# FelipeMartins96/rsoccer-isaac-cleanrl

Measured on AMD Instinct MI355X. Metric: env-steps/s (num_envs×horizon) at 65 536 envs; PPO wall-clock to 1e8 steps, higher is better.
Workload: dtype f32; 1 GPU; vss_step FULL contract: 65536 fields/GPU, one launch per control step, random actions (BASELINE configs[1]/[2] shape); fields_per_gpu=65536, mode=full, agent_rows_per_field=1, launch=eager ctypes launches, parallelism=fields sharded over 1 GPU(s), no data-path collective

## Files before the change

### rsoccer-isaac-cleanrl_amd/csrc/vss_step.hip

```cpp
#include <hip/hip_runtime.h>
#include <type_traits>
#include <stdint.h>

#include "../../include/vss.h"

#pragma clang fp contract(off)

#if defined(__HIP_DEVICE_COMPILE__) && !defined(__gfx950__)
#error "vss_step.hip targets gfx950 (CDNA4) only: wait_loads() and v_permlane32_swap are gfx950 encodings"
#endif

namespace vss {

constexpr int kWave = 64;
constexpr int kFpw = 32;
constexpr int kRec = 59;

constexpr int NSUB = 2;
#define K_H 0.025f
#define K_HH 0.0125f
#define K_FIELD_HX 0.75f
#define K_FIELD_HY 0.65f
#define K_GOAL_HY 0.2f
#define K_GOAL_BACK_X 0.85f
// ... 210 lines not shown
    float dx = ax - K_FIELD_HX, dy = ay - K_GOAL_HY;
    float d2 = dx * dx + dy * dy;
    if (d2 < r * r) {
      float d = sqrtf(d2);
      float nx = -1.0f, ny = 0.0f;
      if (d > 1e-9f) { float inv = 1.0f / d; nx = dx * inv; ny = dy * inv; }
      float pen = r - d;
      ax = ax + nx * pen; ay = ay + ny * pen;
      float vn = avx * nx + avy * ny;
      if (vn < 0.0f) { avx = avx - nx * vn; avy = avy - ny * vn; }
    }
  } else {
    const float px = ax - K_FIELD_HX + r, py = ay - K_GOAL_HY + r;
    const float pen_end = ax + r - K_FIELD_HX, pen_side = ay + r - K_GOAL_HY;
    const bool use_x = in_x || (!in_y && px < py);
    const float pen = in_x ? pen_end : (in_y ? pen_side : (px < py ? px : py));
    push_face(ax, avx, use_x ? pen : -1.0f);
    push_face(ay, avy, use_x ? -1.0f : pen);
  }
  push_face(ay, avy, ay + r - K_FIELD_HY);
  push_face(ax, avx, ax + r - K_GOAL_BACK_X);
  x = ax * sx; y = ay * sy; vx = avx * sx; vy = avy * sy;
}

__device__ __forceinline__ void drive_robot(float c, float s, float& vx, float& vy, float& w, float tl, float tr) {
  float vf = c * vx + s * vy;
  float vl = c * vy - s * vx;
  float wl = vf - w * K_HALF_TRACK;
  float wr = vf + w * K_HALF_TRACK;
  wl = wl + clampf(tl - wl, -K_DV, K_DV);
  wr = wr + clampf(tr - wr, -K_DV, K_DV);
  vf = (wl + wr) * 0.5f;
  w = (wr - wl) * K_INV_TRACK;
  vl = vl - clampf(vl, -K_DL, K_DL);
  vx = c * vf - s * vl;
  vy = s * vf + c * vl;
}

__device__ __forceinline__ void integrate_robot(float& x, float& y, float vx, float vy, float w, float& qz, float& qw,
                                                float& c, float& s) {
  x = x + vx * K_H;
  y = y + vy * K_H;
  float sh, ch;
  sincos_small(w * K_HH, sh, ch);
  const float nqz = qz * ch + qw * sh;
  const float nqw = qw * ch - qz * sh;
  const float k = 1.5f - 0.5f * (nqz * nqz + nqw * nqw);
  qz = nqz * k;
  qw = nqw * k;
  c = qw * qw - qz * qz;
  s = 2.0f * qw * qz;
}

__device__ __forceinline__ void exch(float v, float& lo, float& hi) {
  const auto r = __builtin_amdgcn_permlane32_swap(__float_as_uint(v), __float_as_uint(v), false, false);
  lo = __uint_as_float(r[0]);
  hi = __uint_as_float(r[1]);
}

__device__ __forceinline__ void physics_split(Bodies& b, const float a[12]) {
  const bool up = threadIdx.x >= 32;
  float tl[3], tr[3], ox[3], oy[3], ovx[3], ovy[3], ow[3], oqz[3], oqw[3], oc[3], os[3];
#pragma unroll
  for (int k = 0; k < 3; ++k) {
    const float al = up ? a[2 * k + 6] : a[2 * k], ar = up ? a[2 * k + 7] : a[2 * k + 1];
    tl[k] = (al * K_WHEEL_RAD_S) * K_WHEEL_R;
    tr[k] = (ar * K_WHEEL_RAD_S) * K_WHEEL_R;
    ox[k] = up ? b.x[k + 3] : b.x[k];
    oy[k] = up ? b.y[k + 3] : b.y[k];
    ovx[k] = up ? b.vx[k + 3] : b.vx[k];
    ovy[k] = up ? b.vy[k + 3] : b.vy[k];
    ow[k] = up ? b.w[k + 3] : b.w[k];
    oqz[k] = up ? b.qz[k + 3] : b.qz[k];
    oqw[k] = up ? b.qw[k + 3] : b.qw[k];
    oc[k] = oqw[k] * oqw[k] - oqz[k] * oqz[k];
    os[k] = 2.0f * oqw[k] * oqz[k];
  }
#pragma unroll 1
  for (int sub = 0; sub < NSUB; ++sub) {
#pragma unroll
    for (int k = 0; k < 3; ++k) {
      drive_robot(oc[k], os[k], ovx[k], ovy[k], ow[k], tl[k], tr[k]);
      integrate_robot(ox[k], oy[k], ovx[k], ovy[k], ow[k], oqz[k], oqw[k], oc[k], os[k]);
      exch(ox[k], b.x[k], b.x[k + 3]);
      exch(oy[k], b.y[k], b.y[k + 3]);
      exch(ovx[k], b.vx[k], b.vx[k + 3]);
      exch(ovy[k], b.vy[k], b.vy[k + 3]);
      exch(oc[k], b.c[k], b.c[k + 3]);
      exch(os[k], b.s[k], b.s[k + 3]);
    }
    b.bvx = b.bvx * K_BALL_DAMP;
    b.bvy = b.bvy * K_BALL_DAMP;
    b.bx = b.bx + b.bvx * K_H;
    b.by = b.by + b.bvy * K_H;
#pragma unroll
    for (int i = 0; i < 6; ++i)
#pragma unroll
      for (int j = i + 1; j < 6; ++j) contact_robot_robot(b, i, j);
#pragma unroll
    for (int i = 0; i < 6; ++i) contact_ball_robot(b, i);
#pragma unroll
    for (int k = 0; k < 3; ++k) {
      ox[k] = up ? b.x[k + 3] : b.x[k];
      oy[k] = up ? b.y[k + 3] : b.y[k];
      ovx[k] = up ? b.vx[k + 3] : b.vx[k];
      ovy[k] = up ? b.vy[k + 3] : b.vy[k];
      contact_walls(ox[k], oy[k], ovx[k], ovy[k], K_ROBOT_R);
      exch(ox[k], b.x[k], b.x[k + 3]);
      exch(oy[k], b.y[k], b.y[k + 3]);
      exch(ovx[k], b.vx[k], b.vx[k + 3]);
      exch(ovy[k], b.vy[k], b.vy[k + 3]);
    }
    contact_walls(b.bx, b.by, b.bvx, b.bvy, K_BALL_R);
  }
// ... 61 lines not shown
    const float2* g2 = reinterpret_cast<const float2*>(g);
    for (int q = lane; q < total / 2; q += kWave) {
      float2 v = at(g2, 8u * (uint32_t)q);
      int e = q * 2, fl = e / W, k = e - fl * W;
      float* d = lds + fl * kRec + k;
      d[0] = v.x; d[1] = v.y;
    }
  }
}

template <int W>
__device__ __forceinline__ void coop_store(float* __restrict__ g, int nv, const float* lds, int lane) {
  const int total = nv * W;
  if constexpr (W % 4 == 0) {
    float4* g4 = reinterpret_cast<float4*>(g);
    for (int q = lane; q < total / 4; q += kWave) {
      int e = q * 4, fl = e / W, k = e - fl * W;
      const float* s = lds + fl * kRec + k;
      at(g4, 16u * (uint32_t)q) = make_float4(s[0], s[1], s[2], s[3]);
    }
  } else {
    float2* g2 = reinterpret_cast<float2*>(g);
    for (int q = lane; q < total / 2; q += kWave) {
      int e = q * 2, fl = e / W, k = e - fl * W;
      const float* s = lds + fl * kRec + k;
      at(g2, 8u * (uint32_t)q) = make_float2(s[0], s[1]);
    }
  }
}

template <int A>
__device__ __forceinline__ void write_obs_record(float* rec, const Bodies& b, const float dof[12]) {
  rec[0] = b.bx; rec[1] = b.by; rec[2] = b.bvx; rec[3] = b.bvy;
#pragma unroll
  for (int r = 0; r < 6; ++r) {
    float* o = rec + 4 + 9 * r;
    o[0] = b.x[r]; o[1] = b.y[r]; o[2] = b.vx[r]; o[3] = b.vy[r];
    o[4] = b.qw[r] * b.qw[r] - b.qz[r] * b.qz[r];
    o[5] = 2.0f * b.qw[r] * b.qz[r];
    o[6] = b.w[r]; o[7] = dof[2 * r]; o[8] = dof[2 * r + 1];
  }
  if constexpr (A == 6) {
    float* m = rec + kRec;
#pragma unroll
    for (int k = 0; k < 4; ++k) m[k] = __uint_as_float(__float_as_uint(rec[k]) ^ 0x80000000u);
#pragma unroll
    for (int r = 0; r < 6; ++r)
#pragma unroll
      for (int q = 0; q < 6; ++q)
        m[4 + 6 * r + q] = __uint_as_float(__float_as_uint(rec[4 + 9 * r + q]) ^ 0x80000000u);
  }
}

constexpr int kObsUnroll = 4;
template <int A, int A0 = 0, int REC = obs_rec<A>()>
__device__ __forceinline__ void coop_store_obs(float* __restrict__ out, int nv, const float* lds, const uint32_t* tab,
                                               int lane, bool nt = false) {
  static_assert(A0 + A <= 6 && (A0 == 0 || REC == kRecObs6), "yellow agents read the mirror slots");
  constexpr int Q = 13 * A;
  constexpr int QD = kWave / Q, QR = kWave % Q;
  constexpr uint32_t RB = 4u * REC;
  const int total = nv * Q;
  const uint32_t rb_last = (uint32_t)(nv - 1) * RB;
  int fl = lane / Q, j4 = lane - fl * Q;
  uint32_t rb = (uint32_t)fl * RB;
  const char* L = reinterpret_cast<const char*>(lds);
  float4* o4 = reinterpret_cast<float4*>(out);
  for (int q0 = lane; q0 < total; q0 += kObsUnroll * kWave) {
    float4 v[kObsUnroll];
#pragma unroll
    for (int u = 0; u < kObsUnroll; ++u) {
      const uint2 t = reinterpret_cast<const uint2*>(tab)[13 * A0 + j4];
      const uint32_t r = rb < rb_last ? rb : rb_last;
      v[u].x = *reinterpret_cast<const float*>(L + r + (t.x & 0xffffu));
      v[u].y = *reinterpret_cast<const float*>(L + r + (t.x >> 16));
      v[u].z = *reinterpret_cast<const float*>(L + r + (t.y & 0xffffu));
      v[u].w = *reinterpret_cast<const float*>(L + r + (t.y >> 16));
      j4 += QR;
      rb += QD * RB;
      if (j4 >= Q) { j4 -= Q; rb += RB; }
    }
#pragma unroll
    for (int u = 0; u < kObsUnroll; ++u)
      if (q0 + u * kWave < total) {
        if (nt) {
          typedef float f4v __attribute__((ext_vector_type(4)));
          __builtin_nontemporal_store(f4v{v[u].x, v[u].y, v[u].z, v[u].w},
                                      reinterpret_cast<f4v*>(&at(o4, 16u * (uint32_t)(q0 + u * kWave))));
        } else {
          at(o4, 16u * (uint32_t)(q0 + u * kWave)) = v[u];
        }
      }
  }
}

struct ResetDraws {
  uint32_t k0, k1, field, ctr, ext;
  const float* u;
  uint32_t rounds;
};

template <bool REPLAY>
__device__ __forceinline__ float uval(uint32_t w) { return REPLAY ? __uint_as_float(w) : u01(w); }

template <bool REPLAY>
__device__ __forceinline__ void pos_block(const ResetDraws& d, uint32_t round, uint32_t blk, uint32_t o[4]) {
  if constexpr (REPLAY) {
#pragma unroll
    for (uint32_t i = 0; i < 4; ++i) {
      const uint32_t j = 4u * blk + i;
      o[i] = j < 14u ? __float_as_uint(d.u[14u * round + j]) : 0x3f000000u;
    }
  } else {
    philox(d.k0, d.k1, d.field, d.ctr, ((kPurposePos | d.ext) << 24) | round, blk, o);
  }
}

template <bool REPLAY>
__device__ __forceinline__ void ang_block(const ResetDraws& d, uint32_t rounds_used, uint32_t blk, uint32_t o[4]) {
  if constexpr (REPLAY) {
#pragma unroll
    for (uint32_t i = 0; i < 4; ++i) o[i] = __float_as_uint(d.u[14u * rounds_used + 4u * blk + i]);
  } else {
    philox(d.k0, d.k1, d.field, d.ctr, ((kPurposeAng | d.ext) << 24), blk, o);
  }
}

template <bool REPLAY>
__device__ __forceinline__ void reset_field(Bodies& b, const ResetDraws& d) {
  const float scale_x = 1.5f - 0.14f, scale_y = 1.3f - 0.14f;
  float px[7], py[7];
  uint32_t round = 0;
  for (;; ++round) {
    uint32_t o[16];
#pragma unroll
    for (int blk = 0; blk < 4; ++blk) pos_block<REPLAY>(d, round, (uint32_t)blk, o + 4 * blk);
#pragma unroll
    for (int e = 0; e < 7; ++e) {
      px[e] = (uval<REPLAY>(o[2 * e]) - 0.5f) * scale_x;
      py[e] = (uval<REPLAY>(o[2 * e + 1]) - 0.5f) * scale_y;
    }
    bool close = false;
#pragma unroll
    for (int i = 0; i < 7; ++i)
#pragma unroll
      for (int j = i + 1; j < 7; ++j) {
        float dx = px[i] - px[j], dy = py[i] - py[j];
        close |= dx * dx + dy * dy < __uint_as_float(0x3ba0902du);
      }
    if (!close || round + 1 >= d.rounds) break;
  }
  b.bx = px[0]; b.by = py[0];
  uint32_t o[8];
  ang_block<REPLAY>(d, round + 1, 0u, o);
  ang_block<REPLAY>(d, round + 1, 1u, o + 4);
#pragma unroll
  for (int r = 0; r < 6; ++r) {
    b.x[r] = px[1 + r]; b.y[r] = py[1 + r];
    b.vx[r] = 0.0f; b.vy[r] = 0.0f; b.w[r] = 0.0f;
    float ang = K_TWO_PI * uval<REPLAY>(o[r]) + (-K_PI);
    float sh, ch;
    sincos_small(ang * 0.5f, sh, ch);
    float nrm = sqrtf(sh * sh + ch * ch);
    b.qz[r] = sh / nrm;
    b.qw[r] = ch / nrm;
  }
  b.bvx = uval<REPLAY>(o[6]) - 0.5f;
  b.bvy = uval<REPLAY>(o[7]) - 0.5f;
}

template <bool REPLAY>
__device__ __forceinline__ void reset_field_split(Bodies& b, const ResetDraws& d) {
  const float kMinDist2 = __uint_as_float(0x3ba0902du);
  const bool up = threadIdx.x >= 32;
  const uint32_t blk0 = up ? 2u : 0u;
  const float scale_x = 1.5f - 0.14f, scale_y = 1.3f - 0.14f;
  float px[8], py[8];
  uint32_t round = 0;
  for (;; ++round) {
    uint32_t o[8];
    pos_block<REPLAY>(d, round, blk0, o);
    pos_block<REPLAY>(d, round, blk0 + 1u, o + 4);
#pragma unroll
    for (int e = 0; e < 4; ++e) {
      exch((uval<REPLAY>(o[2 * e]) - 0.5f) * scale_x, px[e], px[4 + e]);
      exch((uval<REPLAY>(o[2 * e + 1]) - 0.5f) * scale_y, py[e], py[4 + e]);
    }
    bool close = false;
#pragma unroll
    for (int i = 0; i < 7; ++i)
#pragma unroll
      for (int j = i + 1; j < 7; ++j) {
        float dx = px[i] - px[j], dy = py[i] - py[j];
        close |= dx * dx + dy * dy < kMinDist2;
      }
    if (!close || round + 1 >= d.rounds) break;
  }
  b.bx = px[0]; b.by = py[0];
  uint32_t oa[4], ang_u[8];
  ang_block<REPLAY>(d, round + 1, up ? 1u : 0u, oa);
#pragma unroll
  for (int i = 0; i < 4; ++i) {
    float lo, hi;
    exch(__uint_as_float(oa[i]), lo, hi);
    ang_u[i] = __float_as_uint(lo);
    ang_u[4 + i] = __float_as_uint(hi);
  }
#pragma unroll
  for (int k = 0; k < 3; ++k) {
    float ang = K_TWO_PI * uval<REPLAY>(up ? ang_u[k + 3] : ang_u[k]) + (-K_PI);
    float sh, ch;
    sincos_small(ang * 0.5f, sh, ch);
    float nrm = sqrtf(sh * sh + ch * ch);
    exch(sh / nrm, b.qz[k], b.qz[k + 3]);
    exch(ch / nrm, b.qw[k], b.qw[k + 3]);
  }
#pragma unroll
  for (int r = 0; r < 6; ++r) {
    b.x[r] = px[1 + r]; b.y[r] = py[1 + r];
    b.vx[r] = 0.0f; b.vy[r] = 0.0f; b.w[r] = 0.0f;
  }
  b.bvx = uval<REPLAY>(ang_u[6]) - 0.5f;
  b.bvy = uval<REPLAY>(ang_u[7]) - 0.5f;
}

__device__ __forceinline__ int64_t rewards_and_done(const vss_params& p, const Bodies& b, float pbx, float pby,
                                                   const float prx[6], const float pry[6], const float a[12],
                                                   int64_t progress, float rew[24]) {
  const float bx = b.bx, by = b.by;
  const bool is_goal = (fabsf(bx) > K_FIELD_HX) && (fabsf(by) < K_GOAL_HY);
  const float g = is_goal ? (bx > 0.0f ? 1.0f : (bx < 0.0f ? -1.0f : 0.0f)) : 0.0f;
  float grad;
  {
    float lx = bx - (-K_FIELD_HX), ly = by - (-0.0f), rx = bx - K_FIELD_HX, ry = by - 0.0f;
    float pot = sqrtf(lx * lx + ly * ly) - sqrtf(rx * rx + ry * ry);
    float plx = pbx - (-K_FIELD_HX), ply = pby - (-0.0f), prx_ = pbx - K_FIELD_HX, pry_ = pby - 0.0f;
    float ppot = sqrtf(plx * plx + ply * ply) - sqrtf(prx_ * prx_ + pry_ * pry_);
    grad = pot - ppot;
  }
#pragma unroll
  for (int ag = 0; ag < 6; ++ag) {
    const bool blue = ag < 3;
    float r0 = 0.0f, r1 = 0.0f, r2 = 0.0f, r3 = 0.0f;
    if (p.w_goal > 0.0f) r0 = (blue ? g : (0.0f - g)) * p.w_goal;
    if (p.w_grad > 0.0f) r1 = (blue ? grad : -grad) * p.w_grad;
    if (p.w_move > 0.0f) {
      float dx0 = prx[ag] - pbx, dy0 = pry[ag] - pby;
      float dx1 = b.x[ag] - bx, dy1 = b.y[ag] - by;
      float pd = sqrtf(dx0 * dx0 + dy0 * dy0), d = sqrtf(dx1 * dx1 + dy1 * dy1);
      r2 = 0.0f + (pd - d) * p.w_move;
    }
    if (p.w_energy > 0.0f)
      r3 = 0.0f + (-((fabsf(a[2 * ag]) + fabsf(a[2 * ag + 1])) / 2.0f)) * p.w_energy;
    rew[4 * ag] = r0; rew[4 * ag + 1] = r1; rew[4 * ag + 2] = r2; rew[4 * ag + 3] = r3;
  }
  return (is_goal || progress >= (int64_t)p.max_episode_length) ? 1 : 0;
}

__device__ __forceinline__ void prefetch12(const float* __restrict__ g, int nv, int lane, float4 pre[3]) {
  const float4* g4 = reinterpret_cast<const float4*>(g);
#pragma unroll
  for (int j = 0; j < 3; ++j) {
    const int q = lane + j * kWave;
    if (q < nv * 3) pre[j] = at(g4, 16u * (uint32_t)q);
  }
}

__device__ __forceinline__ void stage12(const float4 pre[3], int nv, float* lds, int lane) {
#pragma unroll
  for (int j = 0; j < 3; ++j) {
    const int q = lane + j * kWave;
    if (q < nv * 3) {
      const int fl = q / 3, k = (q - fl * 3) * 4;
      float* d = lds + fl * kRec + k;
      d[0] = pre[j].x; d[1] = pre[j].y; d[2] = pre[j].z; d[3] = pre[j].w;
    }
  }
}

template <int NL>
__device__ __forceinline__ void prefetch_lrn(const float* __restrict__ g, int nv, int lane, float2 pre[2]) {
  const float2* g2 = reinterpret_cast<const float2*>(g);
#pragma unroll
  for (int j = 0; j < 2; ++j) {
    const int q = lane + j * kWave;
    if (q < nv * NL / 2) pre[j] = at(g2, 8u * (uint32_t)q);
  }
}

template <int NL>
__device__ __forceinline__ void stage_lrn(const float2 pre[2], int nv, float* lds, int lane) {
#pragma unroll
  for (int j = 0; j < 2; ++j) {
    const int q = lane + j * kWave;
    if (q < nv * NL / 2) {
      const int e = q * 2, fl = e / NL, k = e - fl * NL;
      float* d = lds + fl * kRec + k;
      d[0] = pre[j].x; d[1] = pre[j].y;
    }
  }
}

__device__ __forceinline__ void box_muller(uint32_t w1, uint32_t w2, float& zc, float& zs) {
  const float u1 = u01_open0(w1), u2 = u01(w2);
  const float rad = sqrtf(-2.0f * logf_poly(u1));
  float sz, cz;
  sincos_turn(u2, sz, cz);
  zc = K_OU_SIGMA * (rad * cz);
  zs = K_OU_SIGMA * (rad * sz);
}

template <int MODE>
__device__ __forceinline__ void ou_noise_split(float a[12], uint32_t k0, uint32_t k1, uint32_t field, uint32_t ctr) {
  const bool up = threadIdx.x >= 32;
  float z[12];
  if constexpr (MODE == VSS_MODE_SA) {
    uint32_t p[4], q[4];
    philox(k0, k1, field, ctr, kPurposeOU << 24, up ? 2u : 0u, p);
    philox(k0, k1, field, ctr, kPurposeOU << 24, up ? 2u : 1u, q);
    float c0, s0, c1, s1, c2, s2;
    box_muller(up ? p[0] : p[2], up ? p[1] : p[3], c0, s0);
    box_muller(up ? p[2] : q[0], up ? p[3] : q[1], c1, s1);
    box_muller(q[2], q[3], c2, s2);
    exch(c0, z[2], z[8]);
    exch(s0, z[3], z[9]);
    exch(c1, z[4], z[10]);
    exch(s1, z[5], z[11]);
    float unused;
    exch(c2, z[6], unused);
    exch(s2, z[7], unused);
  } else {
    uint32_t p[4];
    philox(k0, k1, field, ctr, kPurposeOU << 24, up ? 2u : 1u, p);
    float c0, s0, c1, s1;
    box_muller(up ? p[0] : p[2], up ? p[1] : p[3], c0, s0);
    box_muller(p[2], p[3], c1, s1);
    exch(c0, z[6], z[8]);
    exch(s0, z[7], z[9]);
    float unused;
    exch(c1, unused, z[10]);
    exch(s1, unused, z[11]);
  }
  constexpr int NL = MODE == VSS_MODE_SA ? 2 : 6;
#pragma unroll
  for (int k = NL; k < 12; ++k) a[k] = clampf((a[k] - K_OU_THETA * a[k]) + z[k], -1.0f, 1.0f);
}

struct BatchIn {
  int64_t progress, reset_prev;
  uint32_t ctr;
  Bodies b;
  float4 blk[3];
  float2 lrn[2];
};

struct StepArgs {
  int64_t n;
  vss_params p;
  vss_state s;
  vss_step_io io;
  vss_replay_draws rd;
  uint32_t rd_rounds;
  uint32_t nt_obs;
};

template <int MODE>
__device__ __forceinline__ void load_batch(const StepArgs& args, int64_t f0, int nv, int fl, int lane, BatchIn& in) {
  constexpr int NL = MODE == VSS_MODE_SA ? 2 : 6;
  in.progress = 0;
  in.reset_prev = 0;
  in.ctr = 0;
  in.b = {};
  if (fl < nv) {
    in.progress = at(args.s.progress_buf + f0, 8u * (uint32_t)fl);
    in.reset_prev = at(args.s.reset_buf + f0, 8u * (uint32_t)fl);
    in.ctr = at(args.s.rng_counter + f0, 4u * (uint32_t)fl);
    load_bodies(args.s.state, args.n, f0, fl, in.b);
  }
  prefetch12((MODE == VSS_MODE_FULL ? args.io.actions : args.io.ou_buf) + f0 * 12, nv, lane, in.blk);
  if constexpr (MODE != VSS_MODE_FULL) prefetch_lrn<NL>(args.io.actions + f0 * NL, nv, lane, in.lrn);
}

template <int MODE, bool REPLAY = false>
__global__ __launch_bounds__(kWave) void step_kernel(StepArgs args) {
  constexpr int A = MODE == VSS_MODE_FULL ? 6 : (MODE == VSS_MODE_DMA ? 3 : 1);
  constexpr int R = MODE == VSS_MODE_DMA ? 3 : 1;
  constexpr int NL = MODE == VSS_MODE_SA ? 2 : 6;
  static_assert(2 * kFpw == kWave, "two lanes per field");
  constexpr int kLds = 32 * kRec > kFpw * obs_rec<A>() ? 32 * kRec : kFpw * obs_rec<A>();
  static_assert(kFpw * obs_rec<A>() <= kLds, "observation records must fit the LDS block");
  __shared__ float lds[kLds + kTabWords];
  uint32_t* tab = reinterpret_cast<uint32_t*>(lds + kLds);
  stage_obs_table(tab, threadIdx.x);

  const int64_t n = args.n;
  const int lane = threadIdx.x;
  const int fl = lane & 31;
  const bool writer = lane < 32;
  const uint32_t k0 = (uint32_t)args.p.seed, k1 = (uint32_t)(args.p.seed >> 32);
  float* rec = lds + fl * kRec;
  float* orec = lds + lane * obs_rec<A>();

  const int64_t f0 = (int64_t)blockIdx.x * kFpw;
  const int nv = (int)(n - f0 < kFpw ? n - f0 : kFpw);
  BatchIn cur;
  load_batch<MODE>(args, f0, nv, fl, lane, cur);
  const int64_t f = f0 + fl;
  const bool valid = fl < nv;
  const bool owner = valid && writer;

  int64_t progress = cur.progress, reset_prev = cur.reset_prev;
  uint32_t ctr = cur.ctr;
  Bodies b = cur.b;

  float a[12];
  stage12(cur.blk, nv, lds, lane);
  __syncthreads();
#pragma unroll
  for (int k = 0; k < 12; ++k) a[k] = rec[k];
  __syncthreads();

  if constexpr (MODE != VSS_MODE_FULL) {
    if constexpr (REPLAY) {
      if (valid) {
        const float* z = args.rd.normals + f * 12;
#pragma unroll
        for (int k = NL; k < 12; ++k) a[k] = clampf((a[k] - K_OU_THETA * a[k]) + z[k], -1.0f, 1.0f);
      }
    } else {
      ou_noise_split<MODE>(a, k0, k1, (uint32_t)f, ctr);
    }
    stage_lrn<NL>(cur.lrn, nv, lds, lane);
    __syncthreads();
#pragma unroll
    for (int k = 0; k < NL; ++k) a[k] = rec[k];
    __syncthreads();
  }
  float ou[12];
  if constexpr (MODE != VSS_MODE_FULL) {
#pragma unroll
    for (int k = 0; k < 12; ++k) ou[k] = a[k];
  }

  const float clip = args.p.clip_actions;
#pragma unroll
  for (int k = 0; k < 12; ++k) a[k] = clampf(a[k], -clip, clip);
  if (reset_prev != 0) progress = 0;

  float pbx = b.bx, pby = b.by, prx[6], pry[6];
#pragma unroll
  for (int i = 0; i < 6; ++i) { prx[i] = b.x[i]; pry[i] = b.y[i]; }

  if (valid) physics_split(b, a);

  progress += 1;
  float rew[24];
  const int64_t done = rewards_and_done(args.p, b, pbx, pby, prx, pry, a, progress, rew);

  wait_loads();

  if (lane < kFpw) write_obs_record<A>(orec, b, a);
  __syncthreads();
  coop_store_obs<A>(args.io.terminal_obs + f0 * (52 * A), nv, lds, tab, lane, MODE != VSS_MODE_FULL);
  __syncthreads();

  float dof[12];
#pragma unroll
  for (int k = 0; k < 12; ++k) dof[k] = a[k];
  if (valid && done) {
    const ResetDraws rd{k0, k1, (uint32_t)f, ctr, 0u, REPLAY ? args.rd.uniforms + f * args.rd.uniform_stride : nullptr,
                        REPLAY ? args.rd_rounds : (uint32_t)kMaxRejectRounds};
    reset_field_split<REPLAY>(b, rd);
#pragma unroll
    for (int k = 0; k < 12; ++k) dof[k] = dof[k] * 0.0f;
  }

  if (lane < kFpw) write_obs_record<A>(orec, b, dof);
  __syncthreads();
  coop_store_obs<A>(args.io.obs + f0 * (52 * A), nv, lds, tab, lane, MODE != VSS_MODE_FULL || args.nt_obs != 0);
  __syncthreads();

  const uint8_t time_out = (progress >= (int64_t)args.p.max_episode_length - 1) && done != 0;
  if (owner) {
    const uint32_t ufl = (uint32_t)fl;
    store_bodies(args.s.state, n, f0, fl, b);
    at(args.s.progress_buf + f0, 8u * ufl) = progress;
    at(args.s.reset_buf + f0, 8u * ufl) = done;
    at(args.s.rng_counter + f0, 4u * ufl) = ctr + 1u;
#pragma unroll
    for (int k = 0; k < R; ++k) {
      at(args.io.time_outs + f0 * R, (uint32_t)(ufl * R + k)) = time_out;
      at(args.io.progress_f + f0 * R, 4u * (ufl * R + k)) = (float)progress;
    }
    if constexpr (MODE == VSS_MODE_DMA) {
#pragma unroll
      for (int k = 0; k < 3; ++k) at(args.io.dones_rep + f0 * 3, 8u * (ufl * 3 + k)) = done;
    }
  }

  if (writer) {
#pragma unroll
    for (int k = 0; k < 12; ++k) rec[k] = dof[k];
  }
  __syncthreads();
  coop_store<12>(args.s.dof_velocity_buf + f0 * 12, nv, lds, lane);
  __syncthreads();
  if constexpr (MODE != VSS_MODE_FULL) {
    if (writer) {
#pragma unroll
      for (int k = 0; k < 12; ++k) rec[k] = done ? ou[k] * 0.0f : ou[k];
    }
    __syncthreads();
    coop_store<12>(args.io.ou_buf + f0 * 12, nv, lds, lane);
    __syncthreads();
  }

  if constexpr (MODE == VSS_MODE_FULL) {
    if (writer) {
#pragma unroll
      for (int k = 0; k < 24; ++k) rec[k] = rew[k];
    }
    __syncthreads();
    coop_store<24>(args.io.rew + f0 * 24, nv, lds, lane);
    if (owner && args.io.reward_sum) at(args.io.reward_sum + f0, 4u * (uint32_t)fl) = ((rew[0] + rew[1]) + rew[2]) + rew[3];
  } else if constexpr (MODE == VSS_MODE_SA) {
    if (owner) {
      at(reinterpret_cast<float4*>(args.io.rew) + f0, 16u * (uint32_t)fl) = make_float4(rew[0], rew[1], rew[2], rew[3]);
      at(args.io.reward_sum + f0, 4u * (uint32_t)fl) = ((rew[0] + rew[1]) + rew[2]) + rew[3];
    }
  } else if constexpr (MODE == VSS_MODE_CMA) {
    if (owner) {
      float m[4];
#pragma unroll
      for (int c = 0; c < 4; ++c) m[c] = ((rew[c] + rew[4 + c]) + rew[8 + c]) / 3.0f;
      at(reinterpret_cast<float4*>(args.io.rew) + f0, 16u * (uint32_t)fl) = make_float4(m[0], m[1], m[2], m[3]);
      at(args.io.reward_sum + f0, 4u * (uint32_t)fl) = ((m[0] + m[1]) + m[2]) + m[3];
    }
  } else {
    if (writer) {
#pragma unroll
      for (int k = 0; k < 12; ++k) rec[k] = rew[k];
    }
    __syncthreads();
    coop_store<12>(args.io.rew + f0 * 12, nv, lds, lane);
    if (owner) {
#pragma unroll
      for (int ag = 0; ag < 3; ++ag)
        at(args.io.reward_sum + f0 * 3, 4u * ((uint32_t)fl * 3 + ag)) =
            ((rew[4 * ag] + rew[4 * ag + 1]) + rew[4 * ag + 2]) + rew[4 * ag + 3];
    }
  }
}

template <int MODE>
__global__ __launch_bounds__(kWave) void step_versus_kernel(StepArgs args, vss_versus_io vs) {
  static_assert(MODE == VSS_MODE_SA || MODE == VSS_MODE_CMA || MODE == VSS_MODE_DMA, "wrapped modes only");
  constexpr int A = MODE == VSS_MODE_DMA ? 3 : 1;
  constexpr int R = MODE == VSS_MODE_DMA ? 3 : 1;
  constexpr int NL = MODE == VSS_MODE_SA ? 2 : 6;
  static_assert(2 * kFpw == kWave, "two lanes per field");
  constexpr int kLds = 32 * kRec > kFpw * kRecObs6 ? 32 * kRec : kFpw * kRecObs6;
  __shared__ float lds[kLds + kTabWords];
  uint32_t* tab = reinterpret_cast<uint32_t*>(lds + kLds);
  stage_obs_table(tab, threadIdx.x);

  const int64_t n = args.n;
  const int lane = threadIdx.x;
  const int fl = lane & 31;
  const bool writer = lane < 32;
  const uint32_t k0 = (uint32_t)args.p.seed, k1 = (uint32_t)(args.p.seed >> 32);
  float* rec = lds + fl * kRec;
  float* orec = lds + lane * kRecObs6;

  const int64_t f0 = (int64_t)blockIdx.x * kFpw;
  const int nv = (int)(n - f0 < kFpw ? n - f0 : kFpw);
  BatchIn cur;
  load_batch<MODE>(args, f0, nv, fl, lane, cur);
  float2 opp[2];
  prefetch_lrn<6>(vs.opp_actions + f0 * 6, nv, lane, opp);
  const int64_t f = f0 + fl;
  const bool valid = fl < nv;
  const bool owner = valid && writer;

  int64_t progress = cur.progress, reset_prev = cur.reset_prev;
  const uint32_t ctr = cur.ctr;
  Bodies b = cur.b;

  float a[12];
  stage12(cur.blk, nv, lds, lane);
  __syncthreads();
#pragma unroll
  for (int k = 0; k < 12; ++k) a[k] = rec[k];
  __syncthreads();
  if constexpr (MODE == VSS_MODE_SA) {
    const bool up = lane >= 32;
    uint32_t w[4];
    philox(k0, k1, (uint32_t)f, ctr, kPurposeOU << 24, up ? 1u : 0u, w);
    float zc, zs, z[6];
    box_muller(up ? w[0] : w[2], up ? w[1] : w[3], zc, zs);
    exch(zc, z[2], z[4]);
    exch(zs, z[3], z[5]);
#pragma unroll
    for (int k = 2; k < 6; ++k) a[k] = clampf((a[k] - K_OU_THETA * a[k]) + z[k], -1.0f, 1.0f);
  }
// ... 288 lines not shown
                                                          unsigned long long* tally) {
  const int64_t f = (int64_t)blockIdx.x * blockDim.x + threadIdx.x;
  const int lane = threadIdx.x & 63;
  bool done = false;
  int q = 0;
  float goal = 0.0f;
  long long steps = 0;
  if (f < n_fields) {
    const int64_t r = f * rows_per_field;
    done = dones[r] != 0;
    if (done) {
      q = (int)(f / group_fields);
      goal = rew[r].x;
      steps = (long long)progress_f[r];
    }
  }
  unsigned long long todo = __ballot(done);
  while (todo) {
    const int leader = __ffsll(todo) - 1;
    const int qq = __shfl(q, leader);
    const bool mine = done && q == qq;
    const unsigned long long m = __ballot(mine);
    const unsigned long long won = __ballot(mine && goal > 0.0f);
    const unsigned long long lost = __ballot(mine && goal < 0.0f);
    long long s = mine ? steps : 0;
#pragma unroll
    for (int d = 32; d >= 1; d >>= 1) s += __shfl_xor(s, d);
    if (lane == leader) {
      unsigned long long* t = tally + 4 * qq;
      atomicAdd(t + 0, (unsigned long long)__popcll(m));
      if (won) atomicAdd(t + 1, (unsigned long long)__popcll(won));
      if (lost) atomicAdd(t + 2, (unsigned long long)__popcll(lost));
      atomicAdd(t + 3, (unsigned long long)s);
    }
    todo &= ~m;
  }
}

}

static bool bad(const void* ptr, uintptr_t align) { return !ptr || (reinterpret_cast<uintptr_t>(ptr) & (align - 1)); }
static bool misaligned(const void* ptr, uintptr_t align) { return ptr && (reinterpret_cast<uintptr_t>(ptr) & (align - 1)); }

static int check_state(int64_t n, const vss_state* st) {
  if (n < 0 || n > (int64_t(1) << 26) || !st) return VSS_E_ARG;
  if (bad(st->state, 4) || bad(st->progress_buf, 8) || bad(st->reset_buf, 8) || bad(st->dof_velocity_buf, 16) ||
      bad(st->rng_counter, 4))
    return VSS_E_ARG;
  return VSS_OK;
}

static int launch_status() { return hipGetLastError() == hipSuccess ? VSS_OK : VSS_E_LAUNCH; }

static int replay_rounds(const vss_replay_draws* d) {
  if (!d || bad(d->uniforms, 4) || d->uniform_stride < 22 || d->uniform_stride > (int64_t(1) << 20)) return -1;
  const int64_t r = (d->uniform_stride - 8) / 14;
  return r > vss::kMaxRejectRounds ? -1 : (int)r;
}

template <bool REPLAY>
static int step_impl(void* stream, int64_t n, int32_t mode, const vss_params* p, const vss_state* st,
                     const vss_step_io* io, const vss_replay_draws* rd) {
  if (int rc = check_state(n, st)) return rc;
  if (!p || !io || mode < VSS_MODE_FULL || mode > VSS_MODE_DMA) return VSS_E_ARG;
  if (bad(io->actions, mode == VSS_MODE_FULL ? 16 : 8) || bad(io->obs, 16) || bad(io->terminal_obs, 16) ||
      bad(io->rew, 16) || bad(io->time_outs, 1) || bad(io->progress_f, 4) || misaligned(io->reward_sum, 4) ||
      misaligned(io->ou_buf, 16) || misaligned(io->dones_rep, 8))
    return VSS_E_ARG;
  if (mode != VSS_MODE_FULL && (!io->ou_buf || !io->reward_sum)) return VSS_E_ARG;
  if (mode == VSS_MODE_DMA && !io->dones_rep) return VSS_E_ARG;
  int rounds = 0;
  if (REPLAY) {
    rounds = replay_rounds(rd);
    if (rounds < 1 || (mode != VSS_MODE_FULL && bad(rd->normals, 4))) return VSS_E_ARG;
  }
  if (n == 0) return VSS_OK;
  const uint32_t nt_obs = mode == VSS_MODE_FULL && n > (int64_t)(256ll << 20) / 3101 ? 1u : 0u;
  vss::StepArgs args{n, *p, *st, *io, REPLAY ? *rd : vss_replay_draws{}, (uint32_t)rounds, nt_obs};
  const dim3 grid((unsigned)((n + vss::kFpw - 1) / vss::kFpw)), block(vss::kWave);
  hipStream_t s = (hipStream_t)stream;
  switch (mode) {
    case VSS_MODE_FULL: hipLaunchKernelGGL((vss::step_kernel<VSS_MODE_FULL, REPLAY>), grid, block, 0, s, args); break;
    case VSS_MODE_SA: hipLaunchKernelGGL((vss::step_kernel<VSS_MODE_SA, REPLAY>), grid, block, 0, s, args); break;
    case VSS_MODE_CMA: hipLaunchKernelGGL((vss::step_kernel<VSS_MODE_CMA, REPLAY>), grid, block, 0, s, args); break;
    default: hipLaunchKernelGGL((vss::step_kernel<VSS_MODE_DMA, REPLAY>), grid, block, 0, s, args); break;
  }
  return launch_status();
}

extern "C" {

int vss_abi_version(void) { return VSS_ABI_VERSION; }


const char* vss_error_string(int code) {
  switch (code) {
    case VSS_OK: return "ok";
    case VSS_E_ARG: return "invalid argument (null or misaligned buffer, bad size or bad mode)";
    case VSS_E_LAUNCH: return "kernel launch failed";
    default: return "unknown error";
  }
}

int vss_step(void* stream, int64_t n, int32_t mode, const vss_params* p, const vss_state* st,
             const vss_step_io* io) {
  return step_impl<false>(stream, n, mode, p, st, io, nullptr);
}

int vss_step_replay(void* stream, int64_t n, int32_t mode, const vss_params* p, const vss_state* st,
                    const vss_step_io* io, const vss_replay_draws* draws) {
  return step_impl<true>(stream, n, mode, p, st, io, draws);
}

int vss_step_versus(void* stream, int64_t n, int32_t mode, const vss_params* p, const vss_state* st,
                    const vss_step_io* io, const vss_versus_io* vs) {
  if (int rc = check_state(n, st)) return rc;
  if (!p || !io || !vs || mode < VSS_MODE_SA || mode > VSS_MODE_DMA) return VSS_E_ARG;
  if (bad(io->actions, 8) || bad(io->ou_buf, 16) || bad(io->obs, 16) || bad(io->terminal_obs, 16) || bad(io->rew, 16) ||
      bad(io->reward_sum, 4) || bad(io->time_outs, 1) || bad(io->progress_f, 4) || misaligned(io->dones_rep, 8) ||
      bad(vs->opp_actions, 8) || bad(vs->opp_obs, 16))
    return VSS_E_ARG;
  if (mode == VSS_MODE_DMA && !io->dones_rep) return VSS_E_ARG;
  if (n == 0) return VSS_OK;
  vss::StepArgs args{n, *p, *st, *io, vss_replay_draws{}, 0u, 0u};
  const dim3 grid((unsigned)((n + vss::kFpw - 1) / vss::kFpw)), block(vss::kWave);
  hipStream_t s = (hipStream_t)stream;
  switch (mode) {
    case VSS_MODE_SA: hipLaunchKernelGGL((vss::step_versus_kernel<VSS_MODE_SA>), grid, block, 0, s, args, *vs); break;
    case VSS_MODE_CMA: hipLaunchKernelGGL((vss::step_versus_kernel<VSS_MODE_CMA>), grid, block, 0, s, args, *vs); break;
    default: hipLaunchKernelGGL((vss::step_versus_kernel<VSS_MODE_DMA>), grid, block, 0, s, args, *vs); break;
  }
  return launch_status();
}
// ... 79 lines not shown
```

Baseline: 1.699 billion env-steps/s.

## Pack eight field-waves per block and fuse obs stores when no field resets

Adds a FULL-mode kernel with eight independent 64-lane waves per block, each with its own LDS slice. It swaps block barriers for wave-local fences and raises priority on the first half of the waves, chosen when the grid fills all CUs about once. When no field in a wave resets, the observation record is built once and written to both terminal_obs and obs, skipping a second LDS staging pass. Rewards move after the stores and are computed split across the two half-waves via permlane swaps. This adds code paths and relies on wave-level sync being enough within a wave.

```diff
diff --git a/rsoccer-isaac-cleanrl_amd/csrc/vss_step.hip b/rsoccer-isaac-cleanrl_amd/csrc/vss_step.hip
--- a/rsoccer-isaac-cleanrl_amd/csrc/vss_step.hip
+++ b/rsoccer-isaac-cleanrl_amd/csrc/vss_step.hip
@@ -286,6 +286,8 @@
   s = 2.0f * qw * qz;
 }
 
+__device__ __forceinline__ bool upper_half() { return (threadIdx.x & 32u) != 0; }
+
 __device__ __forceinline__ void exch(float v, float& lo, float& hi) {
   const auto r = __builtin_amdgcn_permlane32_swap(__float_as_uint(v), __float_as_uint(v), false, false);
   lo = __uint_as_float(r[0]);
@@ -293,7 +295,7 @@
 }
 
 __device__ __forceinline__ void physics_split(Bodies& b, const float a[12]) {
-  const bool up = threadIdx.x >= 32;
+  const bool up = upper_half();
   float tl[3], tr[3], ox[3], oy[3], ovx[3], ovy[3], ow[3], oqz[3], oqw[3], oc[3], os[3];
 #pragma unroll
   for (int k = 0; k < 3; ++k) {
@@ -461,10 +463,34 @@
   }
 }
 
+__device__ __forceinline__ void write_obs_record_halves(float* rec, const Bodies& b, const float dof[12]) {
+  static_assert(mirror_slot(3) == 3 + kRec && mirror_slot(4 + 9 * 5 + 5) == 4 + 9 * 5 + 5 + kRec - 3 * 5 &&
+                    mirror_slot(4 + 9 * 2) == 4 + 9 * 2 + kRec - 3 * 2,
+                "mirror slot = plain slot + kRec - 3 r");
+  const bool up = upper_half();
+  const uint32_t sgn = up ? 0x80000000u : 0u;
+  float* m = rec + (up ? kRec : 0);
+  m[0] = __uint_as_float(__float_as_uint(b.bx) ^ sgn);
+  m[1] = __uint_as_float(__float_as_uint(b.by) ^ sgn);
+  m[2] = __uint_as_float(__float_as_uint(b.bvx) ^ sgn);
+  m[3] = __uint_as_float(__float_as_uint(b.bvy) ^ sgn);
+#pragma unroll
+  for (int r = 0; r < 6; ++r) {
+    float* o = rec + 4 + 9 * r + (up ? kRec - 3 * r : 0);
+    o[0] = __uint_as_float(__float_as_uint(b.x[r]) ^ sgn);
+    o[1] = __uint_as_float(__float_as_uint(b.y[r]) ^ sgn);
+    o[2] = __uint_as_float(__float_as_uint(b.vx[r]) ^ sgn);
+    o[3] = __uint_as_float(__float_as_uint(b.vy[r]) ^ sgn);
+    o[4] = __uint_as_float(__float_as_uint(b.qw[r] * b.qw[r] - b.qz[r] * b.qz[r]) ^ sgn);
+    o[5] = __uint_as_float(__float_as_uint(2.0f * b.qw[r] * b.qz[r]) ^ sgn);
+    if (!up) { o[6] = b.w[r]; o[7] = dof[2 * r]; o[8] = dof[2 * r + 1]; }
+  }
+}
+
 constexpr int kObsUnroll = 4;
-template <int A, int A0 = 0, int REC = obs_rec<A>()>
+template <int A, int A0 = 0, int REC = obs_rec<A>(), bool DUAL = false>
 __device__ __forceinline__ void coop_store_obs(float* __restrict__ out, int nv, const float* lds, const uint32_t* tab,
-                                               int lane, bool nt = false) {
+                                               int lane, bool nt = false, float* __restrict__ out2 = nullptr) {
   static_assert(A0 + A <= 6 && (A0 == 0 || REC == kRecObs6), "yellow agents read the mirror slots");
   constexpr int Q = 13 * A;
   constexpr int QD = kWave / Q, QR = kWave % Q;
@@ -475,6 +501,7 @@
   uint32_t rb = (uint32_t)fl * RB;
   const char* L = reinterpret_cast<const char*>(lds);
   float4* o4 = reinterpret_cast<float4*>(out);
+  float4* p4 = reinterpret_cast<float4*>(DUAL ? out2 : out);
   for (int q0 = lane; q0 < total; q0 += kObsUnroll * kWave) {
     float4 v[kObsUnroll];
 #pragma unroll
@@ -492,12 +519,13 @@
 #pragma unroll
     for (int u = 0; u < kObsUnroll; ++u)
       if (q0 + u * kWave < total) {
+        if constexpr (DUAL) at(o4, 16u * (uint32_t)(q0 + u * kWave)) = v[u];
         if (nt) {
           typedef float f4v __attribute__((ext_vector_type(4)));
           __builtin_nontemporal_store(f4v{v[u].x, v[u].y, v[u].z, v[u].w},
-                                      reinterpret_cast<f4v*>(&at(o4, 16u * (uint32_t)(q0 + u * kWave))));
+                                      reinterpret_cast<f4v*>(&at(p4, 16u * (uint32_t)(q0 + u * kWave))));
         } else {
-          at(o4, 16u * (uint32_t)(q0 + u * kWave)) = v[u];
+          at(p4, 16u * (uint32_t)(q0 + u * kWave)) = v[u];
         }
       }
   }
@@ -581,7 +609,7 @@
 template <bool REPLAY>
 __device__ __forceinline__ void reset_field_split(Bodies& b, const ResetDraws& d) {
   const float kMinDist2 = __uint_as_float(0x3ba0902du);
-  const bool up = threadIdx.x >= 32;
+  const bool up = upper_half();
   const uint32_t blk0 = up ? 2u : 0u;
   const float scale_x = 1.5f - 0.14f, scale_y = 1.3f - 0.14f;
   float px[8], py[8];
@@ -631,6 +659,55 @@
   }
   b.bvx = uval<REPLAY>(ang_u[6]) - 0.5f;
   b.bvy = uval<REPLAY>(ang_u[7]) - 0.5f;
+}
+
+__device__ __forceinline__ bool ball_in_goal(float bx, float by) {
+  return (fabsf(bx) > K_FIELD_HX) && (fabsf(by) < K_GOAL_HY);
+}
+
+__device__ __forceinline__ int64_t done_flag(const vss_params& p, const Bodies& b, int64_t progress) {
+  return (ball_in_goal(b.bx, b.by) || progress >= (int64_t)p.max_episode_length) ? 1 : 0;
+}
+
+__device__ __forceinline__ float goal_potential(float x, float y) {
+  float lx = x - (-K_FIELD_HX), ly = y - (-0.0f), rx = x - K_FIELD_HX, ry = y - 0.0f;
+  return sqrtf(lx * lx + ly * ly) - sqrtf(rx * rx + ry * ry);
+}
+
+__device__ __forceinline__ float move_reward(float px, float py, float pbx, float pby, float x, float y, float bx,
+                                             float by, float w_move) {
+  float dx0 = px - pbx, dy0 = py - pby;
+  float dx1 = x - bx, dy1 = y - by;
+  float pd = sqrtf(dx0 * dx0 + dy0 * dy0), d = sqrtf(dx1 * dx1 + dy1 * dy1);
+  return 0.0f + (pd - d) * w_move;
+}
+
+__device__ __forceinline__ void rewards_split(const vss_params& p, float bx, float by, const float x[6],
+                                              const float y[6], float pbx, float pby, const float prx[6],
+                                              const float pry[6], const float a[12], float rew[24]) {
+  const bool up = upper_half();
+  const float g = ball_in_goal(bx, by) ? (bx > 0.0f ? 1.0f : (bx < 0.0f ? -1.0f : 0.0f)) : 0.0f;
+  float pot, ppot, mv[6];
+  exch(goal_potential(up ? pbx : bx, up ? pby : by), pot, ppot);
+  const float grad = pot - ppot;
+  if (p.w_move > 0.0f) {
+#pragma unroll
+    for (int k = 0; k < 3; ++k)
+      exch(move_reward(up ? prx[k + 3] : prx[k], up ? pry[k + 3] : pry[k], pbx, pby, up ? x[k + 3] : x[k],
+                       up ? y[k + 3] : y[k], bx, by, p.w_move),
+           mv[k], mv[k + 3]);
+  }
+#pragma unroll
+  for (int ag = 0; ag < 6; ++ag) {
+    const bool blue = ag < 3;
+    float r0 = 0.0f, r1 = 0.0f, r2 = 0.0f, r3 = 0.0f;
+    if (p.w_goal > 0.0f) r0 = (blue ? g : (0.0f - g)) * p.w_goal;
+    if (p.w_grad > 0.0f) r1 = (blue ? grad : -grad) * p.w_grad;
+    if (p.w_move > 0.0f) r2 = mv[ag];
+    if (p.w_energy > 0.0f)
+      r3 = 0.0f + (-((fabsf(a[2 * ag]) + fabsf(a[2 * ag + 1])) / 2.0f)) * p.w_energy;
+    rew[4 * ag] = r0; rew[4 * ag + 1] = r1; rew[4 * ag + 2] = r2; rew[4 * ag + 3] = r3;
+  }
 }
 
 __device__ __forceinline__ int64_t rewards_and_done(const vss_params& p, const Bodies& b, float pbx, float pby,
@@ -721,7 +798,7 @@
 
 template <int MODE>
 __device__ __forceinline__ void ou_noise_split(float a[12], uint32_t k0, uint32_t k1, uint32_t field, uint32_t ctr) {
-  const bool up = threadIdx.x >= 32;
+  const bool up = upper_half();
   float z[12];
   if constexpr (MODE == VSS_MODE_SA) {
     uint32_t p[4], q[4];
@@ -790,27 +867,54 @@
   if constexpr (MODE != VSS_MODE_FULL) prefetch_lrn<NL>(args.io.actions + f0 * NL, nv, lane, in.lrn);
 }
 
-template <int MODE, bool REPLAY = false>
-__global__ __launch_bounds__(kWave) void step_kernel(StepArgs args) {
+template <int MODE>
+constexpr int step_lds_floats() {
+  constexpr int A = MODE == VSS_MODE_FULL ? 6 : (MODE == VSS_MODE_DMA ? 3 : 1);
+  return (32 * kRec > kFpw * obs_rec<A>() ? 32 * kRec : kFpw * obs_rec<A>()) + kTabWords;
+}
+
+constexpr int kPairWaves = 8;
+
+template <int WPB>
+__device__ __forceinline__ void wave_sync() {
+  if constexpr (WPB == 1) {
+    __syncthreads();
+  } else {
+    __builtin_amdgcn_fence(__ATOMIC_ACQ_REL, "wavefront");
+    __builtin_amdgcn_s_waitcnt(0xC07F);
+    __builtin_amdgcn_wave_barrier();
+  }
+}
+
+template <int MODE, bool REPLAY, int WPB>
+__device__ __forceinline__ void step_body(const StepArgs& args, float* lds) {
   constexpr int A = MODE == VSS_MODE_FULL ? 6 : (MODE == VSS_MODE_DMA ? 3 : 1);
   constexpr int R = MODE == VSS_MODE_DMA ? 3 : 1;
   constexpr int NL = MODE == VSS_MODE_SA ? 2 : 6;
   static_assert(2 * kFpw == kWave, "two lanes per field");
-  constexpr int kLds = 32 * kRec > kFpw * obs_rec<A>() ? 32 * kRec : kFpw * obs_rec<A>();
+  static_assert(WPB == 1 || MODE == VSS_MODE_FULL, "the paired shape is FULL's");
+  constexpr int kLds = step_lds_floats<MODE>() - kTabWords;
   static_assert(kFpw * obs_rec<A>() <= kLds, "observation records must fit the LDS block");
-  __shared__ float lds[kLds + kTabWords];
+  const int64_t n = args.n;
+  const int wave = WPB == 1 ? 0 : (int)(threadIdx.x >> 6);
+  const int lane = WPB == 1 ? (int)threadIdx.x : (int)(threadIdx.x & 63u);
+  const bool first = WPB > 1 && wave < WPB / 2;
+  if constexpr (WPB > 1) {
+    if (first) __builtin_amdgcn_s_setprio(3);
+  }
+  const int64_t f0 = ((int64_t)blockIdx.x * WPB + wave) * kFpw;
+  if constexpr (WPB > 1) {
+    if (f0 >= n) return;
+  }
   uint32_t* tab = reinterpret_cast<uint32_t*>(lds + kLds);
-  stage_obs_table(tab, threadIdx.x);
-
-  const int64_t n = args.n;
-  const int lane = threadIdx.x;
+  stage_obs_table(tab, lane);
+
   const int fl = lane & 31;
   const bool writer = lane < 32;
   const uint32_t k0 = (uint32_t)args.p.seed, k1 = (uint32_t)(args.p.seed >> 32);
   float* rec = lds + fl * kRec;
   float* orec = lds + lane * obs_rec<A>();
 
-  const int64_t f0 = (int64_t)blockIdx.x * kFpw;
   const int nv = (int)(n - f0 < kFpw ? n - f0 : kFpw);
   BatchIn cur;
   load_batch<MODE>(args, f0, nv, fl, lane, cur);
@@ -824,10 +928,10 @@
 
   float a[12];
   stage12(cur.blk, nv, lds, lane);
-  __syncthreads();
+  wave_sync<WPB>();
 #pragma unroll
   for (int k = 0; k < 12; ++k) a[k] = rec[k];
-  __syncthreads();
+  wave_sync<WPB>();
 
   if constexpr (MODE != VSS_MODE_FULL) {
     if constexpr (REPLAY) {
@@ -840,10 +944,10 @@
       ou_noise_split<MODE>(a, k0, k1, (uint32_t)f, ctr);
     }
     stage_lrn<NL>(cur.lrn, nv, lds, lane);
-    __syncthreads();
+    wave_sync<WPB>();
 #pragma unroll
     for (int k = 0; k < NL; ++k) a[k] = rec[k];
-    __syncthreads();
+    wave_sync<WPB>();
   }
   float ou[12];
   if constexpr (MODE != VSS_MODE_FULL) {
@@ -863,31 +967,64 @@
   if (valid) physics_split(b, a);
 
   progress += 1;
+  constexpr bool kShortHead = MODE == VSS_MODE_FULL;
   float rew[24];
-  const int64_t done = rewards_and_done(args.p, b, pbx, pby, prx, pry, a, progress, rew);
+  int64_t done;
+  if constexpr (kShortHead) done = done_flag(args.p, b, progress);
+  else done = rewards_and_done(args.p, b, pbx, pby, prx, pry, a, progress, rew);
 
   wait_loads();
 
-  if (lane < kFpw) write_obs_record<A>(orec, b, a);
-  __syncthreads();
-  coop_store_obs<A>(args.io.terminal_obs + f0 * (52 * A), nv, lds, tab, lane, MODE != VSS_MODE_FULL);
-  __syncthreads();
-
   float dof[12];
 #pragma unroll
   for (int k = 0; k < 12; ++k) dof[k] = a[k];
-  if (valid && done) {
-    const ResetDraws rd{k0, k1, (uint32_t)f, ctr, 0u, REPLAY ? args.rd.uniforms + f * args.rd.uniform_stride : nullptr,
-                        REPLAY ? args.rd_rounds : (uint32_t)kMaxRejectRounds};
-    reset_field_split<REPLAY>(b, rd);
-#pragma unroll
-    for (int k = 0; k < 12; ++k) dof[k] = dof[k] * 0.0f;
-  }
-
-  if (lane < kFpw) write_obs_record<A>(orec, b, dof);
-  __syncthreads();
-  coop_store_obs<A>(args.io.obs + f0 * (52 * A), nv, lds, tab, lane, MODE != VSS_MODE_FULL || args.nt_obs != 0);
-  __syncthreads();
+  const ResetDraws rd{k0, k1, (uint32_t)f, ctr, 0u, REPLAY ? args.rd.uniforms + f * args.rd.uniform_stride : nullptr,
+                      REPLAY ? args.rd_rounds : (uint32_t)kMaxRejectRounds};
+  if constexpr (kShortHead) {
+    const float qbx = b.bx, qby = b.by;
+    float qx[6], qy[6];
+#pragma unroll
+    for (int i = 0; i < 6; ++i) { qx[i] = b.x[i]; qy[i] = b.y[i]; }
+    float* frec = lds + fl * kRecObs6;
+    const bool nt = args.nt_obs != 0;
+    write_obs_record_halves(frec, b, a);
+    wave_sync<WPB>();
+    if (__ballot(valid && done != 0) == 0) {
+      coop_store_obs<6, 0, kRecObs6, true>(args.io.terminal_obs + f0 * 312, nv, lds, tab, lane, nt,
+                                           args.io.obs + f0 * 312);
+      if (first) __builtin_amdgcn_s_setprio(0);
+    } else {
+      coop_store_obs<6>(args.io.terminal_obs + f0 * 312, nv, lds, tab, lane, false);
+      if (first) __builtin_amdgcn_s_setprio(0);
+      wave_sync<WPB>();
+      if (valid && done) {
+        reset_field_split<REPLAY>(b, rd);
+#pragma unroll
+        for (int k = 0; k < 12; ++k) dof[k] = dof[k] * 0.0f;
+      }
+      write_obs_record_halves(frec, b, dof);
+      wave_sync<WPB>();
+      coop_store_obs<6>(args.io.obs + f0 * 312, nv, lds, tab, lane, nt);
+    }
+    wave_sync<WPB>();
+    rewards_split(args.p, qbx, qby, qx, qy, pbx, pby, prx, pry, a, rew);
+  } else {
+    if (lane < kFpw) write_obs_record<A>(orec, b, a);
+    wave_sync<WPB>();
+    coop_store_obs<A>(args.io.terminal_obs + f0 * (52 * A), nv, lds, tab, lane, true);
+    wave_sync<WPB>();
+
+    if (valid && done) {
+      reset_field_split<REPLAY>(b, rd);
+#pragma unroll
+      for (int k = 0; k < 12; ++k) dof[k] = dof[k] * 0.0f;
+    }
+
+    if (lane < kFpw) write_obs_record<A>(orec, b, dof);
+    wave_sync<WPB>();
+    coop_store_obs<A>(args.io.obs + f0 * (52 * A), nv, lds, tab, lane, true);
+    wave_sync<WPB>();
+  }
 
   const uint8_t time_out = (progress >= (int64_t)args.p.max_episode_length - 1) && done != 0;
   if (owner) {
@@ -911,17 +1048,17 @@
 #pragma unroll
     for (int k = 0; k < 12; ++k) rec[k] = dof[k];
   }
-  __syncthreads();
+  wave_sync<WPB>();
   coop_store<12>(args.s.dof_velocity_buf + f0 * 12, nv, lds, lane);
-  __syncthreads();
+  wave_sync<WPB>();
   if constexpr (MODE != VSS_MODE_FULL) {
     if (writer) {
 #pragma unroll
       for (int k = 0; k < 12; ++k) rec[k] = done ? ou[k] * 0.0f : ou[k];
     }
-    __syncthreads();
+    wave_sync<WPB>();
     coop_store<12>(args.io.ou_buf + f0 * 12, nv, lds, lane);
-    __syncthreads();
+    wave_sync<WPB>();
   }
 
   if constexpr (MODE == VSS_MODE_FULL) {
@@ -929,7 +1066,7 @@
 #pragma unroll
       for (int k = 0; k < 24; ++k) rec[k] = rew[k];
     }
-    __syncthreads();
+    wave_sync<WPB>();
     coop_store<24>(args.io.rew + f0 * 24, nv, lds, lane);
     if (owner && args.io.reward_sum) at(args.io.reward_sum + f0, 4u * (uint32_t)fl) = ((rew[0] + rew[1]) + rew[2]) + rew[3];
   } else if constexpr (MODE == VSS_MODE_SA) {
@@ -950,7 +1087,7 @@
 #pragma unroll
       for (int k = 0; k < 12; ++k) rec[k] = rew[k];
     }
-    __syncthreads();
+    wave_sync<WPB>();
     coop_store<12>(args.io.rew + f0 * 12, nv, lds, lane);
     if (owner) {
 #pragma unroll
@@ -959,6 +1096,17 @@
             ((rew[4 * ag] + rew[4 * ag + 1]) + rew[4 * ag + 2]) + rew[4 * ag + 3];
     }
   }
+}
+
+template <int MODE, bool REPLAY = false>
+__global__ __launch_bounds__(kWave) void step_kernel(StepArgs args) {
+  __shared__ float lds[step_lds_floats<MODE>()];
+  step_body<MODE, REPLAY, 1>(args, lds);
+}
+
+__global__ __launch_bounds__(kWave* kPairWaves) void step_full_paired_kernel(StepArgs args) {
+  extern __shared__ float paired_lds[];
+  step_body<VSS_MODE_FULL, false, kPairWaves>(args, paired_lds + (threadIdx.x >> 6) * step_lds_floats<VSS_MODE_FULL>());
 }
 
 template <int MODE>
@@ -1353,6 +1501,23 @@
 
 static int launch_status() { return hipGetLastError() == hipSuccess ? VSS_OK : VSS_E_LAUNCH; }
 
+constexpr int kPairedLdsBytes = vss::kPairWaves * vss::step_lds_floats<VSS_MODE_FULL>() * (int)sizeof(float);
+static int paired_cus() {
+  constexpr int kMaxDev = 64;
+  static int cus[kMaxDev];
+  int dev = 0;
+  if (hipGetDevice(&dev) != hipSuccess || dev < 0 || dev >= kMaxDev) return 0;
+  if (cus[dev] == 0) {
+    int count = 0;
+    const bool ok = hipDeviceGetAttribute(&count, hipDeviceAttributeMultiprocessorCount, dev) == hipSuccess && count > 0 &&
+                    hipFuncSetAttribute(reinterpret_cast<const void*>(vss::step_full_paired_kernel),
+                                        hipFuncAttributeMaxDynamicSharedMemorySize, kPairedLdsBytes) == hipSuccess;
+    if (!ok) (void)hipGetLastError();
+    cus[dev] = ok ? count : -1;
+  }
+  return cus[dev] > 0 ? cus[dev] : 0;
+}
+
 static int replay_rounds(const vss_replay_draws* d) {
   if (!d || bad(d->uniforms, 4) || d->uniform_stride < 22 || d->uniform_stride > (int64_t(1) << 20)) return -1;
   const int64_t r = (d->uniform_stride - 8) / 14;
@@ -1380,6 +1545,15 @@
   vss::StepArgs args{n, *p, *st, *io, REPLAY ? *rd : vss_replay_draws{}, (uint32_t)rounds, nt_obs};
   const dim3 grid((unsigned)((n + vss::kFpw - 1) / vss::kFpw)), block(vss::kWave);
   hipStream_t s = (hipStream_t)stream;
+  if (!REPLAY && mode == VSS_MODE_FULL && !nt_obs) {
+    const int cus = paired_cus();
+    const int64_t waves = grid.x;
+    if (cus > 0 && waves > (int64_t)(vss::kPairWaves - 1) * cus && waves <= (int64_t)vss::kPairWaves * cus) {
+      const dim3 pgrid((unsigned)((waves + vss::kPairWaves - 1) / vss::kPairWaves)), pblock(vss::kWave * vss::kPairWaves);
+      hipLaunchKernelGGL(vss::step_full_paired_kernel, pgrid, pblock, kPairedLdsBytes, s, args);
+      return launch_status();
+    }
+  }
   switch (mode) {
     case VSS_MODE_FULL: hipLaunchKernelGGL((vss::step_kernel<VSS_MODE_FULL, REPLAY>), grid, block, 0, s, args); break;
     case VSS_MODE_SA: hipLaunchKernelGGL((vss::step_kernel<VSS_MODE_SA, REPLAY>), grid, block, 0, s, args); break;
```

Result: no change. 1.712 billion env-steps/s, median of 3 (+0.8%).
